# YuliangXiu/ICON

Measured on NVIDIA H100. Metric: M query-points/sec at 256^3 grid, higher is better.
Workload: dtype f32

## Files before the change

icon_b200/csrc/face_tree.cuh:

```cuda
#pragma once
#include <float.h>

#include "common.cuh"
#include "geom.cuh"

namespace icon {

__device__ __forceinline__ float box_dist2(V3 p, float4 lo, float4 hi) {
    const float dx = fmaxf(fmaxf(lo.x - p.x, p.x - hi.x), 0.f);
    const float dy = fmaxf(fmaxf(lo.y - p.y, p.y - hi.y), 0.f);
    const float dz = fmaxf(fmaxf(lo.z - p.z, p.z - hi.z), 0.f);
    return fmaf(dz, dz, fmaf(dy, dy, dx * dx));
}
__device__ __forceinline__ float box_far2(V3 p, float4 lo, float4 hi) {
    const float dx = fmaxf(fabsf(lo.x - p.x), fabsf(hi.x - p.x));
    const float dy = fmaxf(fabsf(lo.y - p.y), fabsf(hi.y - p.y));
    const float dz = fmaxf(fabsf(lo.z - p.z), fabsf(hi.z - p.z));
    return fmaf(dz, dz, fmaf(dy, dy, dx * dx));
}
__device__ __forceinline__ float warp_max(float v) {
    for (int o = 16; o; o >>= 1) v = fmaxf(v, __shfl_xor_sync(0xffffffffu, v, o));
    return v;
}
__device__ __forceinline__ float warp_min(float v) {
    for (int o = 16; o; o >>= 1) v = fminf(v, __shfl_xor_sync(0xffffffffu, v, o));
    return v;
}

static inline size_t tree_levels(FaceTree &t, int F) {
    t.F = F;
    int n = (F + 3) / 4, o = 0, l = 0;
    while (true) {
        t.lvl_cnt[l] = n; t.lvl_off[l] = o; o += n; ++l;
        if (n == 1) break;
        n = (n + 3) / 4;
    }
    t.nlevels = l;
    return (size_t)o;
}

__device__ __forceinline__ unsigned expand10(unsigned v) {
    v = (v * 0x00010001u) & 0xFF0000FFu;
    v = (v * 0x00000101u) & 0x0F00F00Fu;
    v = (v * 0x00000011u) & 0xC30C30C3u;
    v = (v * 0x00000005u) & 0x49249249u;
    return v;
}

__device__ __forceinline__ unsigned morton30(V3 p, V3 lo, float s) {
    auto qz = [s](float v, float l) { return (unsigned)fminf(fmaxf((v - l) * s, 0.f), 1023.f); };
    return (expand10(qz(p.x, lo.x)) << 2) | (expand10(qz(p.y, lo.y)) << 1) | expand10(qz(p.z, lo.z));
}

__device__ __forceinline__ V3 write_face_record(V3 a, V3 b, V3 c, float slack, float4 *__restrict__ tri,
                                                float4 *__restrict__ sph) {
    const V3 ab = sub3(b, a), ac = sub3(c, a);
    const V3 sc = mk3((a.x + b.x + c.x) / 3.f, (a.y + b.y + c.y) / 3.f, (a.z + b.z + c.z) / 3.f);
    const float ra = dot3(sub3(a, sc), sub3(a, sc)), rb = dot3(sub3(b, sc), sub3(b, sc)),
                rc = dot3(sub3(c, sc), sub3(c, sc));
    const float sr = sqrtf(fmaxf(ra, fmaxf(rb, rc))) * 1.0001f + slack;
    tri[0] = make_float4(a.x, a.y, a.z, ab.x);
    tri[1] = make_float4(ab.y, ab.z, ac.x, ac.y);
    tri[2] = make_float4(ac.z, 0.f, 0.f, 0.f);
    *sph = make_float4(sc.x, sc.y, sc.z, sr);
    return sc;
}

__device__ __forceinline__ void write_leaf_box(const FaceTree &t, int n) {
    float4 lo = make_float4(FLT_MAX, FLT_MAX, FLT_MAX, 0.f), hi = make_float4(-FLT_MAX, -FLT_MAX, -FLT_MAX, 0.f);
    for (int k = 4 * n; k < min(4 * n + 4, t.F); ++k) {
        const Tri tr = load_tri(t.tri_s + 3 * (size_t)k);
        const V3 vs[3] = {tr.a, mk3(tr.a.x + tr.ab.x, tr.a.y + tr.ab.y, tr.a.z + tr.ab.z),
                          mk3(tr.a.x + tr.ac.x, tr.a.y + tr.ac.y, tr.a.z + tr.ac.z)};
        for (int j = 0; j < 3; ++j) {
            lo.x = fminf(lo.x, vs[j].x); hi.x = fmaxf(hi.x, vs[j].x);
            lo.y = fminf(lo.y, vs[j].y); hi.y = fmaxf(hi.y, vs[j].y);
            lo.z = fminf(lo.z, vs[j].z); hi.z = fmaxf(hi.z, vs[j].z);
        }
    }
    t.nodes[2 * (size_t)n] = lo;
    t.nodes[2 * (size_t)n + 1] = hi;
}

__device__ __forceinline__ void write_parent_box(const FaceTree &t, int l, int n) {
    const float4 *child = t.nodes + 2 * (size_t)t.lvl_off[l - 1];
    float4 lo = make_float4(FLT_MAX, FLT_MAX, FLT_MAX, 0.f), hi = make_float4(-FLT_MAX, -FLT_MAX, -FLT_MAX, 0.f);
    for (int c = 4 * n; c < min(4 * n + 4, t.lvl_cnt[l - 1]); ++c) {
        const float4 a = child[2 * (size_t)c], b = child[2 * (size_t)c + 1];
        lo.x = fminf(lo.x, a.x); lo.y = fminf(lo.y, a.y); lo.z = fminf(lo.z, a.z);
        hi.x = fmaxf(hi.x, b.x); hi.y = fmaxf(hi.y, b.y); hi.z = fmaxf(hi.z, b.z);
    }
    t.nodes[2 * ((size_t)t.lvl_off[l] + n)] = lo;
    t.nodes[2 * ((size_t)t.lvl_off[l] + n) + 1] = hi;
}

struct ChunkSmem {
    float4 sph[32];
    float4 tri[32][3];
    int kk[32];
};
template <typename Id, int CAP>
struct WalkSmem : ChunkSmem {
    Id fr[2][CAP];
};

template <int PPW>
struct NearestFace {
    static constexpr int REP = 32 / PPW;
    const int lane;
    V3 p;
    float tol, tol_sup;
    float best = FLT_MAX;
    int bi = 0x7fffffff;
    float sb = 0.f, ub = 0.f;
    int staged = 0;

    __device__ __forceinline__ NearestFace(V3 p_, float tol_, float tol_sup_)
        : lane(threadIdx.x & 31), p(p_), tol(tol_), tol_sup(tol_sup_) {}

    __device__ __forceinline__ float sphere_bound(float d) const {
        const float b = d * rsqrtf(d) * 1.00001f + tol;
        return d > 0.f ? b : tol;
    }

    __device__ __forceinline__ void try_face(const float4 *rec, int f) {
        const Tri tr = load_tri(rec);
        const float d = tri_sqdist(p, tr.a, tr.ab, tr.ac);
        if (d < best || (d == best && f < bi)) { best = d; bi = f; }
    }

    __device__ __forceinline__ void descend(const FaceTree &t, V3 c) {
        int node = 0;
        for (int lvl = t.nlevels - 1; lvl > 0; --lvl) {
            const int ch = 4 * node + (lane & 3);
            float a = FLT_MAX;
            int ai = ch;
            if (ch < t.lvl_cnt[lvl - 1]) {
                const float4 *nb = t.nodes + 2 * ((size_t)t.lvl_off[lvl - 1] + ch);
                a = box_dist2(c, __ldg(nb), __ldg(nb + 1));
            }
            for (int o = 1; o <= 2; o <<= 1) {
                const float ob = __shfl_xor_sync(0xffffffffu, a, o);
                const int oi = __shfl_xor_sync(0xffffffffu, ai, o);
                if (ob < a || (ob == a && oi < ai)) { a = ob; ai = oi; }
            }
            node = __shfl_sync(0xffffffffu, ai, 0);
        }
        for (int k = 4 * node; k < min(4 * node + 4, t.F); ++k) try_face(t.tri_s + 3 * (size_t)k, __ldg(t.order + k));
    }

    __device__ __forceinline__ void start_scan(float ubw) {
        sb = sphere_bound(best);
        ub = ubw * 1.00001f + tol;
    }

    __device__ __forceinline__ void test(const FaceTree &t, int k, float4 s, const float4 *tr) {
        const float dx = p.x - s.x, dy = p.y - s.y, dz = p.z - s.z;
        const float dd = fmaf(dz, dz, fmaf(dy, dy, dx * dx));
        const float l = sb + s.w;
        if (dd > l * l) return;
        const float4 r0 = tr[0], r1 = tr[1], r2 = tr[2];
        const V3 ab = mk3(r0.w, r1.x, r1.y), ac = mk3(r1.z, r1.w, r2.x);
        const float S1 = fmaf(dz, ab.z, fmaf(dy, ab.y, dx * ab.x));
        const float T1 = fmaf(dz, ac.z, fmaf(dy, ac.y, dx * ac.x));
        const float M = fmaxf(fmaxf(-(S1 + T1), fmaf(2.f, S1, -T1)), fmaf(2.f, T1, -S1)) * (1.f / 3.f);
        const float g = dd - M - tol_sup;
        if (g > 0.f && g * g > best * dd * 1.0001f) return;
        const float d = tri_sqdist(p, mk3(r0.x, r0.y, r0.z), ab, ac);
        if (!(d <= best)) return;
        const int f = __ldg(t.order + k);
        if (d < best || f < bi) { best = d; bi = f; sb = sphere_bound(d); }
    }

    __device__ __forceinline__ void merge() {
#pragma unroll
        for (int o = PPW; o < 32; o <<= 1) {
            const float ob = __shfl_xor_sync(0xffffffffu, best, o);
            const int oi = __shfl_xor_sync(0xffffffffu, bi, o);
            if (ob < best || (ob == best && oi < bi)) { best = ob; bi = oi; }
        }
    }

    __device__ __forceinline__ void chunk(const FaceTree &t, ChunkSmem &S, int leaf, float4 wlo, float4 whi) {
        bool pass = false;
        int k = 0;
        float4 s = make_float4(0.f, 0.f, 0.f, 0.f);
        if (leaf >= 0) {
            k = 4 * leaf + (lane & 3);
            if (k < t.F) {
                s = __ldg(t.sph_s + k);
                const float l2 = ub + s.w;
                pass = box_dist2(mk3(s.x, s.y, s.z), wlo, whi) <= l2 * l2;
            }
        }
        const unsigned mask = __ballot_sync(0xffffffffu, pass);
        const int cnt = __popc(mask);
        staged += cnt;
        if (pass) {
            const int at = __popc(mask & ((1u << lane) - 1u));
            const float4 *tp = t.tri_s + 3 * (size_t)k;
            S.sph[at] = s;
            S.kk[at] = k;
            S.tri[at][0] = __ldg(tp); S.tri[at][1] = __ldg(tp + 1); S.tri[at][2] = __ldg(tp + 2);
        }
        __syncwarp();
        for (int j = lane / PPW; j < cnt; j += REP) test(t, S.kk[j], S.sph[j], &S.tri[j][0]);
        if (REP > 1) {
            merge();
            sb = sphere_bound(best);
        }
        ub = fminf(ub, warp_max(sb));
        __syncwarp();
    }

    template <typename Id>
    __device__ __forceinline__ void scan_leaves(const FaceTree &t, ChunkSmem &S, const Id *leaves, int n, float4 wlo,
                                                float4 whi) {
        for (int base = 0; base < n; base += 8) {
            const int slot = base + (lane >> 2);
            chunk(t, S, slot < n ? (int)leaves[slot] : -1, wlo, whi);
        }
    }

    __device__ __forceinline__ void scan_all(const FaceTree &t) {
        for (int k = lane / PPW; k < t.F; k += REP) test(t, k, __ldg(t.sph_s + k), t.tri_s + 3 * (size_t)k);
    }
};

template <typename Id, int CAP>
__device__ __forceinline__ bool tree_cull(const FaceTree &t, Id (&fr)[2][CAP], V3 c, float rw, float4 wlo, float4 whi,
                                          float tol, float &ubw, int &cur, int &n) {
    const int lane = threadIdx.x & 31;
    float ub2 = (ubw * 1.00001f + tol) * (ubw * 1.00001f + tol);
    cur = 0; n = 1;
    bool overflow = false;
    if (lane == 0) fr[0][0] = 0;
    __syncwarp();
    for (int lvl = t.nlevels - 1; lvl > 0 && !overflow; --lvl) {
        int nn = 0;
        float far2 = FLT_MAX;
        const int ccnt = t.lvl_cnt[lvl - 1];
        const float4 *nodes = t.nodes + 2 * (size_t)t.lvl_off[lvl - 1];
        for (int base = 0; base < n; base += 8) {
            const int slot = base + (lane >> 2);
            bool pass = false;
            int ch = 0;
            if (slot < n) {
                ch = 4 * (int)fr[cur][slot] + (lane & 3);
                if (ch < ccnt) {
                    const float4 lo = __ldg(nodes + 2 * (size_t)ch), hi = __ldg(nodes + 2 * (size_t)ch + 1);
                    const float gx = fmaxf(fmaxf(lo.x - whi.x, wlo.x - hi.x), 0.f);
                    const float gy = fmaxf(fmaxf(lo.y - whi.y, wlo.y - hi.y), 0.f);
                    const float gz = fmaxf(fmaxf(lo.z - whi.z, wlo.z - hi.z), 0.f);
                    pass = fmaf(gz, gz, fmaf(gy, gy, gx * gx)) <= ub2;
                    far2 = fminf(far2, box_far2(c, lo, hi));
                }
            }
            const unsigned mask = __ballot_sync(0xffffffffu, pass);
            const int at = nn + __popc(mask & ((1u << lane) - 1u));
            if (pass && at < CAP) fr[cur ^ 1][at] = (Id)ch;
            nn += __popc(mask);
        }
        overflow = nn > CAP;
        n = nn;
        cur ^= 1;
        const float l2 = sqrtf(warp_min(far2)) + rw;
        if (l2 < ubw) { ubw = l2; ub2 = (ubw * 1.00001f + tol) * (ubw * 1.00001f + tol); }
        __syncwarp();
    }
    return !overflow;
}

template <int PPW, typename Id, int CAP>
__device__ __forceinline__ int tree_nearest(const FaceTree &t, WalkSmem<Id, CAP> &S, NearestFace<PPW> &q, V3 c,
                                            float rw, float4 wlo, float4 whi) {
    q.descend(t, c);
    float ubw = warp_max(sqrtf(q.best));
    int cur, n;
    const bool ok = tree_cull(t, S.fr, c, rw, wlo, whi, q.tol, ubw, cur, n);
    q.start_scan(ubw);
    if (ok) q.scan_leaves(t, S, S.fr[cur], n, wlo, whi);
    else q.scan_all(t);
    q.merge();
    return n;
}

}
```

icon_b200/csrc/sdf.cu:

```cuda
#include <float.h>

#include <algorithm>
#include <mutex>
#include <type_traits>
#include <unordered_set>

#include "common.cuh"
#include "face_tree.cuh"
#include "geom.cuh"

namespace icon {

struct Calib {
    float r[9];
    float t[3];
};

__device__ __forceinline__ V3 load_point(const float *__restrict__ pts, int64_t sc, int64_t sn,
                                         int64_t i, const Calib &cb) {
    float px = pts[i * sn], py = pts[sc + i * sn], pz = pts[2 * sc + i * sn];
    V3 o;
    o.x = fmaf(cb.r[2], pz, fmaf(cb.r[1], py, cb.r[0] * px)) + cb.t[0];
    o.y = fmaf(cb.r[5], pz, fmaf(cb.r[4], py, cb.r[3] * px)) + cb.t[1];
    o.z = fmaf(cb.r[8], pz, fmaf(cb.r[7], py, cb.r[6] * px)) + cb.t[2];
    return o;
}

__device__ __forceinline__ void emit_record(V3 p, int bi, float best, int hits, const MeshView &m,
                                            float *__restrict__ rec, int32_t *__restrict__ face,
                                            int64_t idx) {
    Tri t = load_tri(m.tri + 3 * (size_t)bi);
    V3 n = cross3(t.ab, t.ac);
    float s = n.x * n.x + n.y * n.y + n.z * n.z;
    if (s == 0.f) s = 1e-6f;
    float inv = 1.0f / s;
    V3 w = sub3(p, t.a);
    V3 uw = cross3(t.ab, w), wv = cross3(w, t.ac);
    float b2 = (uw.x * n.x + uw.y * n.y + uw.z * n.z) * inv;
    float b1 = (wv.x * n.x + wv.y * n.y + wv.z * n.z) * inv;
    float b0 = 1.0f - b1 - b2;
    const float4 *at = m.attr + 6 * (size_t)bi;
    float4 a0 = __ldg(at), a1 = __ldg(at + 1), a2 = __ldg(at + 2), a3 = __ldg(at + 3),
           a4 = __ldg(at + 4), a5 = __ldg(at + 5);
    float nx = (a0.x * b0 + a0.w * b1 + a1.z * b2) * -1.f;
    float ny = (a0.y * b0 + a1.x * b1 + a1.w * b2) * 1.f;
    float nz = (a0.z * b0 + a1.y * b1 + a2.x * b2) * -1.f;
    float cx = a2.y * b0 + a3.x * b1 + a3.w * b2;
    float cy = a2.z * b0 + a3.y * b1 + a4.x * b2;
    float cz = a2.w * b0 + a3.z * b1 + a4.y * b2;
    float vv = a4.z * b0 + a4.w * b1 + a5.x * b2;
    float vis = vv >= 0.1f ? 1.f : 0.f;
    float dist = sqrtf(best) / sqrtf(3.0f);
    float sign = 2.0f * ((float)(hits & 1) - 0.5f);
    float sdf = dist * sign;
    float4 *r = (float4 *)(rec + 8 * idx);
    r[0] = make_float4(sdf, cx, cy, cz);
    r[1] = make_float4(nx, ny, nz, vis);
    if (face) face[idx] = bi;
}

constexpr int SW_T = 128;
constexpr int NBIN_AX = 128;
constexpr int NBIN = NBIN_AX * NBIN_AX * NBIN_AX;
__host__ __device__ constexpr int fr_cap(int ppw) { return ppw >= 16 ? 1024 : (ppw >= 4 ? 768 : 384); }

__device__ __forceinline__ unsigned spread7(unsigned v) {
    v = (v | (v << 16)) & 0x030000FFu;
    v = (v | (v << 8)) & 0x0300F00Fu;
    v = (v | (v << 4)) & 0x030C30C3u;
    v = (v | (v << 2)) & 0x09249249u;
    return v;
}

__device__ __forceinline__ int bin_of(V3 p) {
    const bool inside = p.x >= -1.f && p.x <= 1.f && p.y >= -1.f && p.y <= 1.f && p.z >= -1.f && p.z <= 1.f;
    if (!inside) return NBIN;
    const unsigned bx = min(NBIN_AX - 1, (int)((p.x + 1.f) * (NBIN_AX * 0.5f)));
    const unsigned by = min(NBIN_AX - 1, (int)((p.y + 1.f) * (NBIN_AX * 0.5f)));
    const unsigned bz = min(NBIN_AX - 1, (int)((p.z + 1.f) * (NBIN_AX * 0.5f)));
    return (int)(spread7(bx) | (spread7(by) << 1) | (spread7(bz) << 2));
}

__global__ void k_points_bin(const float *__restrict__ pts, int64_t sc, int64_t sn, int64_t N, Calib cb,
                             float4 *__restrict__ xyz4, int32_t *__restrict__ bid, int32_t *__restrict__ count) {
    const int64_t i = (int64_t)blockIdx.x * blockDim.x + threadIdx.x;
    const bool live = i < N;
    int b = -1;
    if (live) {
        const V3 p = load_point(pts, sc, sn, i, cb);
        const float in_cube = (p.x > -1.f && p.x < 1.f && p.y > -1.f && p.y < 1.f && p.z > -1.f && p.z < 1.f) ? 1.f : 0.f;
        xyz4[i] = make_float4(p.x, p.y, p.z, in_cube);
        b = bin_of(p);
        bid[i] = b;
    }
    const unsigned act = __ballot_sync(0xffffffffu, live);
    if (live) {
        const unsigned peers = __match_any_sync(act, b);
        if ((int)(threadIdx.x & 31) == __ffs(peers) - 1) atomicAdd(&count[b], __popc(peers));
    }
}

__global__ void k_points_scatter(const int32_t *__restrict__ bid, int64_t N, const int32_t *__restrict__ offset,
                                 int32_t *__restrict__ cursor, int32_t *__restrict__ perm) {
    const int64_t i = (int64_t)blockIdx.x * blockDim.x + threadIdx.x;
    const bool live = i < N;
    const int b = live ? bid[i] : -1;
    const unsigned act = __ballot_sync(0xffffffffu, live);
    if (live) {
        const unsigned peers = __match_any_sync(act, b);
        const int lane = threadIdx.x & 31, leader = __ffs(peers) - 1;
        int base = 0;
        if (lane == leader) base = atomicAdd(&cursor[b], __popc(peers));
        base = __shfl_sync(peers, base, leader);
        perm[offset[b] + base + __popc(peers & ((1u << lane) - 1u))] = (int32_t)i;
    }
}

#ifdef ICON_SDF_STATS
__device__ unsigned long long g_stats[8];
#define STAT(i, v) do { if (lane == 0) atomicAdd(&g_stats[i], (unsigned long long)(v)); } while (0)
#else
#define STAT(i, v) do { } while (0)
#endif

template <int PPW, bool BRICK>
using SdfSmem = typename std::conditional<BRICK, ChunkSmem, WalkSmem<unsigned short, fr_cap(PPW)>>::type;
template <int PPW, bool BRICK>
constexpr size_t sdf_smem_bytes() { return sizeof(SdfSmem<PPW, BRICK>) * (SW_T / 32); }

constexpr float BRICK_W = 2.0f / BRICK_AX;
constexpr float BRICK_HALF_DIAG = 0.0541266f;

__device__ __forceinline__ void brick_box(int b, float4 &lo, float4 &hi) {
    const int bx = b % BRICK_AX, by = (b / BRICK_AX) % BRICK_AX, bz = b / (BRICK_AX * BRICK_AX);
    lo = make_float4(-1.f + bx * BRICK_W, -1.f + by * BRICK_W, -1.f + bz * BRICK_W, 0.f);
    hi = make_float4(-1.f + (bx + 1) * BRICK_W, -1.f + (by + 1) * BRICK_W, -1.f + (bz + 1) * BRICK_W, 0.f);
}

__device__ __forceinline__ float leaf_key(const MeshView &m, int l, float4 lo, float4 hi) {
    const float4 a = __ldg(m.nodes + 2 * (size_t)l), z = __ldg(m.nodes + 2 * (size_t)l + 1);
    const float gx = fmaxf(fmaxf(a.x - hi.x, lo.x - z.x), 0.f);
    const float gy = fmaxf(fmaxf(a.y - hi.y, lo.y - z.y), 0.f);
    const float gz = fmaxf(fmaxf(a.z - hi.z, lo.z - z.z), 0.f);
    return fmaf(gz, gz, fmaf(gy, gy, gx * gx));
}

template <int PPW, bool BRICK>
__device__ __forceinline__ void sdf_warp(int64_t wid, SdfSmem<PPW, BRICK> &S, const float4 *__restrict__ xyz4,
                                         const int32_t *__restrict__ perm, int64_t N, const MeshView &m,
                                         float *__restrict__ rec, int32_t *__restrict__ face,
                                         int32_t *__restrict__ defer, int32_t *__restrict__ ndefer) {
    constexpr int REP = 32 / PPW;
    const int lane = threadIdx.x & 31;
    const int sub = lane % PPW, rep_id = lane / PPW;
    const int64_t pos0 = wid * PPW;
    const int64_t pos = pos0 + sub;
    if (pos0 >= N) return;
    const bool live = pos < N;
    const int64_t idx = perm[live ? pos : pos0];
    const float4 q = xyz4[idx];
    const V3 p = mk3(q.x, q.y, q.z);
    const V3 c = mk3(0.5f * (warp_min(p.x) + warp_max(p.x)), 0.5f * (warp_min(p.y) + warp_max(p.y)),
                     0.5f * (warp_min(p.z) + warp_max(p.z)));
    const float rw = warp_max(sqrtf(dot3(sub3(p, c), sub3(p, c)))) * 1.00001f + 1e-6f;
    const float4 wlo = make_float4(warp_min(p.x) - 1e-6f, warp_min(p.y) - 1e-6f, warp_min(p.z) - 1e-6f, 0.f);
    const float4 whi = make_float4(warp_max(p.x) + 1e-6f, warp_max(p.y) + 1e-6f, warp_max(p.z) + 1e-6f, 0.f);
    const MeshHeader h = *m.hdr;

    NearestFace<PPW> nf(p, 1e-6f, 1e-7f);
    if constexpr (BRICK) {
        bool ok = h.brick_built && !h.brick_overflow && c.x >= -1.f && c.x < 1.f && c.y >= -1.f && c.y < 1.f &&
                  c.z >= -1.f && c.z < 1.f;
        int b = 0;
        float4 blo, bhi;
        if (ok) {
            const int bx = min(BRICK_AX - 1, (int)((c.x + 1.f) * (BRICK_AX * 0.5f)));
            const int by = min(BRICK_AX - 1, (int)((c.y + 1.f) * (BRICK_AX * 0.5f)));
            const int bz = min(BRICK_AX - 1, (int)((c.z + 1.f) * (BRICK_AX * 0.5f)));
            b = (bz * BRICK_AX + by) * BRICK_AX + bx;
            brick_box(b, blo, bhi);
            ok = wlo.x >= blo.x && wlo.y >= blo.y && wlo.z >= blo.z && whi.x <= bhi.x && whi.y <= bhi.y && whi.z <= bhi.z;
        }
        if (!ok) {
            if (lane == 0) defer[atomicAdd(ndefer, 1)] = (int32_t)wid;
            return;
        }
        const int f = __ldg(m.bface + b);
        nf.try_face(m.tri + 3 * (size_t)f, f);
        nf.start_scan(fminf(warp_max(sqrtf(nf.best)), __ldg(m.bub + b)));
        STAT(0, 1);
        const int o1 = __ldg(m.boff + b + 1);
        for (int base = __ldg(m.boff + b); base < o1; base += 8) {
            const int slot = base + (lane >> 2);
            const int leaf = slot < o1 ? (int)__ldg(m.blist + slot) : -1;
            float key = 0.f;
            if (lane == 0) key = leaf_key(m, leaf, blo, bhi);
            if (__shfl_sync(0xffffffffu, key, 0) > nf.ub * nf.ub) break;
            STAT(2, min(8, o1 - base));
            nf.chunk(m, S, leaf, wlo, whi);
        }
        nf.merge();
    } else {
        const int n = tree_nearest(m, S, nf, c, rw, wlo, whi);
        STAT(0, 1); STAT(1, n > fr_cap(PPW) ? 1 : 0); STAT(2, n);
    }
    STAT(3, nf.staged);
    int hits = 0;
    if (!h.ray_overflow) {
        const float fy = (p.y - h.y0) * h.inv_cy, fz = (p.z - h.z0) * h.inv_cz;
        if (fy >= 0.f && fy < (float)RAY_GRID && fz >= 0.f && fz < (float)RAY_GRID) {
            const int cc = (int)fz * RAY_GRID + (int)fy;
            const int k0 = __ldg(m.roff + cc), k1 = __ldg(m.roff + cc + 1);
            for (int k = k0 + rep_id; k < k1; k += REP) {
                const int f = __ldg(m.rlist + k);
                if (__ldg(&m.rbox[2 * (size_t)f + 1].x) < p.x - 1e-3f) continue;
                const Tri tr = load_tri(m.tri + 3 * (size_t)f);
                hits += ray_hit_px(p, tr.a, tr.ab, tr.ac);
            }
        }
    } else {
        for (int f = rep_id; f < m.F; f += REP) {
            const Tri tr = load_tri(m.tri + 3 * (size_t)f);
            hits += ray_hit_px(p, tr.a, tr.ab, tr.ac);
        }
    }
    if (REP > 1) {
#pragma unroll
        for (int o = PPW; o < 32; o <<= 1) hits += __shfl_xor_sync(0xffffffffu, hits, o);
    }
    if (live && rep_id == 0) emit_record(p, nf.bi, nf.best, hits, m, rec, face, idx);
}

template <int PPW, bool BRICK>
__global__ void __launch_bounds__(SW_T) k_sdf_warp(const float4 *__restrict__ xyz4, const int32_t *__restrict__ perm,
                                                   int64_t N, MeshView m, float *__restrict__ rec,
                                                   int32_t *__restrict__ face, int32_t *__restrict__ defer,
                                                   int32_t *__restrict__ ndefer) {
    static_assert(!BRICK || PPW == 32, "brick lists serve dense lattices: 32 points per warp");
    extern __shared__ __align__(16) unsigned char smem_raw[];
    SdfSmem<PPW, BRICK> &S = reinterpret_cast<SdfSmem<PPW, BRICK> *>(smem_raw)[threadIdx.x >> 5];
    const bool listed = !BRICK && defer != nullptr;
    const int64_t nw = listed ? (int64_t)*ndefer : (N + PPW - 1) / PPW;
    for (int64_t i = (int64_t)blockIdx.x * (SW_T / 32) + (threadIdx.x >> 5); i < nw; i += (int64_t)gridDim.x * (SW_T / 32))
        sdf_warp<PPW, BRICK>(listed ? (int64_t)defer[i] : i, S, xyz4, perm, N, m, rec, face, defer, ndefer);
}

__global__ void k_brick_centres(MeshView m) {
    const int b = blockIdx.x * blockDim.x + threadIdx.x;
    if (b >= NBRICK) return;
    float4 lo, hi;
    brick_box(b, lo, hi);
    m.bxyz[b] = make_float4(0.5f * (lo.x + hi.x), 0.5f * (lo.y + hi.y), 0.5f * (lo.z + hi.z), 0.f);
    m.bperm[b] = b;
}

__global__ void __launch_bounds__(128) k_brick_count(MeshView m) {
    __shared__ int s_cnt;
    const int b = blockIdx.x;
    float4 lo, hi;
    brick_box(b, lo, hi);
    const float4 cc = m.bxyz[b];
    const Tri t = load_tri(m.tri + 3 * (size_t)m.bface[b]);
    const float d = tri_sqdist(mk3(cc.x, cc.y, cc.z), t.a, t.ab, t.ac);
    const float ub = (sqrtf(d) + BRICK_HALF_DIAG) * 1.00001f + 1e-6f, ub2 = ub * ub;
    if (threadIdx.x == 0) s_cnt = 0;
    __syncthreads();
    int cnt = 0;
    for (int l = threadIdx.x; l < m.lvl_cnt[0]; l += blockDim.x) cnt += leaf_key(m, l, lo, hi) <= ub2;
    for (int o = 16; o; o >>= 1) cnt += __shfl_xor_sync(0xffffffffu, cnt, o);
    if ((threadIdx.x & 31) == 0) atomicAdd(&s_cnt, cnt);
    __syncthreads();
    if (threadIdx.x == 0) {
        m.bub[b] = ub;
        m.boff[b] = s_cnt;
        if (s_cnt > BRICK_MAX_LEAVES) m.hdr->brick_overflow = 1;
        if (b == 0) m.boff[NBRICK] = 0;
    }
}

__global__ void __launch_bounds__(128) k_brick_fill(MeshView m, int64_t cap) {
    __shared__ float s_key[BRICK_MAX_LEAVES];
    __shared__ unsigned short s_leaf[BRICK_MAX_LEAVES];
    __shared__ int s_wcnt[4];
    if (m.hdr->brick_overflow || m.boff[NBRICK] > cap) return;
    const int b = blockIdx.x, o0 = m.boff[b], lane = threadIdx.x & 31, wib = threadIdx.x >> 5;
    float4 lo, hi;
    brick_box(b, lo, hi);
    const float ub = m.bub[b], ub2 = ub * ub;
    const int nleaf = m.lvl_cnt[0];
    int n = 0;
    for (int l0 = 0; l0 < nleaf; l0 += 128) {
        const int l = l0 + threadIdx.x;
        float key = 0.f;
        if (l < nleaf) key = leaf_key(m, l, lo, hi);
        const bool in = l < nleaf && key <= ub2;
        const unsigned bal = __ballot_sync(0xffffffffu, in);
        if (lane == 0) s_wcnt[wib] = __popc(bal);
        __syncthreads();
        int at = n + __popc(bal & ((1u << lane) - 1u));
        for (int w = 0; w < wib; ++w) at += s_wcnt[w];
        if (in) { s_key[at] = key; s_leaf[at] = (unsigned short)l; }
        n += s_wcnt[0] + s_wcnt[1] + s_wcnt[2] + s_wcnt[3];
        __syncthreads();
    }
    for (int i = threadIdx.x; i < n; i += blockDim.x) {
        const float k = s_key[i];
        int r = 0;
        for (int j = 0; j < n; ++j) {
            const float kj = s_key[j];
            r += kj < k || (kj == k && j < i);
        }
        m.blist[o0 + r] = s_leaf[i];
    }
}

__global__ void k_brick_done(MeshView m, int64_t cap) {
    if (m.boff[NBRICK] > cap) m.hdr->brick_overflow = 1;
    m.hdr->brick_built = 1;
}

__global__ void __launch_bounds__(256) k_sdf_brute(const float *__restrict__ pts, int64_t sc, int64_t sn,
                                                   int64_t N, Calib cb, MeshView m,
                                                   float *__restrict__ rec, int32_t *__restrict__ face) {
    __shared__ float4 tile[3 * 256];
    int64_t i = (int64_t)blockIdx.x * blockDim.x + threadIdx.x;
    bool live = i < N;
    V3 p = mk3(0.f, 0.f, 0.f);
    if (live) p = load_point(pts, sc, sn, i, cb);
    float best = FLT_MAX;
    int bi = 0, hits = 0;
    for (int f0 = 0; f0 < m.F; f0 += 256) {
        int nf = min(256, m.F - f0);
        __syncthreads();
        for (int k = threadIdx.x; k < 3 * nf; k += 256) tile[k] = m.tri[3 * (size_t)f0 + k];
        __syncthreads();
        if (live) {
            for (int k = 0; k < nf; ++k) {
                float4 r0 = tile[3 * k], r1 = tile[3 * k + 1], r2 = tile[3 * k + 2];
                V3 a = mk3(r0.x, r0.y, r0.z), ab = mk3(r0.w, r1.x, r1.y), ac = mk3(r1.z, r1.w, r2.x);
                float d = tri_sqdist(p, a, ab, ac);
                if (d < best) { best = d; bi = f0 + k; }
                hits += ray_hit_px(p, a, ab, ac);
            }
        }
    }
    if (live) emit_record(p, bi, best, hits, m, rec, face, i);
}

static int64_t g_sdf_ppw32_from = 6000000, g_sdf_ppw8_from = 300000;
static int g_sdf_ppw_force = 0;
static int g_sdf_bricks = 1;
static int64_t g_brick_max_entries = 0;

static std::mutex g_brick_mu;
static std::unordered_set<const void *> g_brick_ready;
static int64_t g_brick_builds = 0;

void bricks_forget(const MeshView &m) {
    std::lock_guard<std::mutex> lk(g_brick_mu);
    g_brick_ready.erase(m.hdr);
}

struct SdfWs {
    float4 *xyz4;
    int32_t *bid, *perm, *count, *offset;
    int32_t *defer, *ndefer;
    void *scan_ws;
};
static SdfWs carve_sdf(Carver &c, int64_t N) {
    SdfWs w;
    w.xyz4 = c.take<float4>((size_t)N);
    w.bid = c.take<int32_t>((size_t)N);
    w.perm = c.take<int32_t>((size_t)N);
    w.count = c.take<int32_t>(NBIN + 1);
    w.offset = c.take<int32_t>(NBIN + 1);
    w.defer = c.take<int32_t>((size_t)(N + 31) / 32);
    w.ndefer = c.take<int32_t>(1);
    w.scan_ws = c.take<char>(scan_ws_bytes(NBIN + 1));
    return w;
}

static int build_bricks(const MeshView &m, cudaStream_t stream) {
    const int64_t cap = g_brick_max_entries > 0 ? std::min(g_brick_max_entries, m.brick_cap) : m.brick_cap;
    k_brick_centres<<<NBRICK / 256, 256, 0, stream>>>(m);
    ICON_LAUNCHED();
    k_sdf_warp<1, false><<<NBRICK / (SW_T / 32), SW_T, sdf_smem_bytes<1, false>(), stream>>>(
        m.bxyz, m.bperm, NBRICK, m, m.brec, m.bface, nullptr, nullptr);
    ICON_LAUNCHED();
    k_brick_count<<<NBRICK, 128, 0, stream>>>(m);
    ICON_LAUNCHED();
    int rc = scan_exclusive_i32(m.boff, m.boff, NBRICK + 1, nullptr, m.scan_ws, stream);
    if (rc) return rc;
    k_brick_fill<<<NBRICK, 128, 0, stream>>>(m, cap);
    ICON_LAUNCHED();
    k_brick_done<<<1, 1, 0, stream>>>(m, cap);
    ICON_LAUNCHED();
    return ICON_OK;
}
size_t sdf_ws_bytes(int64_t N) {
    Carver c(nullptr);
    carve_sdf(c, N);
    return c.total();
}

Calib make_calib(const float *h) {
    Calib cb;
    for (int r = 0; r < 3; ++r) {
        for (int k = 0; k < 3; ++k) cb.r[3 * r + k] = h[4 * r + k];
        cb.t[r] = h[4 * r + 3];
    }
    return cb;
}

int run_sdf(const float *points, int64_t sc, int64_t sn, int64_t N, const float *h_calib,
            const MeshView &m, float *rec, int32_t *face, void *ws, float4 **xyz4_out,
            cudaStream_t stream) {
    Carver c(ws);
    SdfWs w = carve_sdf(c, N);
    Calib cb = make_calib(h_calib);
    profile_mark(0, stream);
    ICON_CUDA(cudaMemsetAsync(w.count, 0, sizeof(int32_t) * (NBIN + 1), stream));
    const unsigned nblk = (unsigned)((N + 255) / 256);
    k_points_bin<<<nblk, 256, 0, stream>>>(points, sc, sn, N, cb, w.xyz4, w.bid, w.count);
    ICON_LAUNCHED();
    int rc = scan_exclusive_i32(w.count, w.offset, NBIN + 1, nullptr, w.scan_ws, stream);
    if (rc) return rc;
    ICON_CUDA(cudaMemsetAsync(w.count, 0, sizeof(int32_t) * (NBIN + 1), stream));
    k_points_scatter<<<nblk, 256, 0, stream>>>(w.bid, N, w.offset, w.count, w.perm);
    ICON_LAUNCHED();
    static bool attr_set[ICON_MAX_DEVICES] = {};
    if (device_needs_setup(attr_set)) {
#define ICON_SDF_ATTR(P, B) ICON_CUDA(cudaFuncSetAttribute(k_sdf_warp<P, B>, cudaFuncAttributeMaxDynamicSharedMemorySize, \
                                                           (int)sdf_smem_bytes<P, B>()))
        ICON_SDF_ATTR(32, true); ICON_SDF_ATTR(32, false); ICON_SDF_ATTR(16, false); ICON_SDF_ATTR(8, false);
        ICON_SDF_ATTR(4, false); ICON_SDF_ATTR(2, false); ICON_SDF_ATTR(1, false);
#undef ICON_SDF_ATTR
    }
    profile_mark(1, stream);
    int ppw = N >= g_sdf_ppw32_from ? 32 : (N >= g_sdf_ppw8_from ? 8 : 1);
    if (g_sdf_ppw_force) ppw = g_sdf_ppw_force;
    const int wpb = SW_T / 32;
    const int64_t nwarps = (N + ppw - 1) / ppw;
    const unsigned nblk_w = (unsigned)((nwarps + wpb - 1) / wpb);
#define ICON_SDF_LAUNCH(P) k_sdf_warp<P, false><<<nblk_w, SW_T, sdf_smem_bytes<P, false>(), stream>>>( \
        w.xyz4, w.perm, N, m, rec, face, nullptr, nullptr)
    if (ppw == 32 && g_sdf_bricks) {
        bool build;
        {
            std::lock_guard<std::mutex> lk(g_brick_mu);
            build = g_brick_ready.insert(m.hdr).second;
        }
        if (build) {
            rc = build_bricks(m, stream);
            std::lock_guard<std::mutex> lk(g_brick_mu);
            if (rc) { g_brick_ready.erase(m.hdr); return rc; }
            ++g_brick_builds;
        }
        ICON_CUDA(cudaMemsetAsync(w.ndefer, 0, sizeof(int32_t), stream));
        k_sdf_warp<32, true><<<nblk_w, SW_T, sdf_smem_bytes<32, true>(), stream>>>(
            w.xyz4, w.perm, N, m, rec, face, w.defer, w.ndefer);
        ICON_LAUNCHED();
        const unsigned nblk_d = (unsigned)std::min<int64_t>(nblk_w, (int64_t)device_sm_count() * 16);
        k_sdf_warp<32, false><<<nblk_d, SW_T, sdf_smem_bytes<32, false>(), stream>>>(
            w.xyz4, w.perm, N, m, rec, face, w.defer, w.ndefer);
    } else {
        switch (ppw) {
            case 32: ICON_SDF_LAUNCH(32); break;
            case 16: ICON_SDF_LAUNCH(16); break;
            case 8: ICON_SDF_LAUNCH(8); break;
            case 4: ICON_SDF_LAUNCH(4); break;
            case 2: ICON_SDF_LAUNCH(2); break;
            default: ICON_SDF_LAUNCH(1); break;
        }
    }
#undef ICON_SDF_LAUNCH
    ICON_LAUNCHED();
    profile_mark(2, stream);
    if (xyz4_out) *xyz4_out = w.xyz4;
    return ICON_OK;
}

__global__ void k_points_only(const float *__restrict__ pts, int64_t sc, int64_t sn, int64_t N, Calib cb,
                              float4 *__restrict__ xyz4) {
    int64_t i = (int64_t)blockIdx.x * blockDim.x + threadIdx.x;
    if (i >= N) return;
    V3 p = load_point(pts, sc, sn, i, cb);
    float in_cube = (p.x > -1.f && p.x < 1.f && p.y > -1.f && p.y < 1.f && p.z > -1.f && p.z < 1.f) ? 1.f : 0.f;
    xyz4[i] = make_float4(p.x, p.y, p.z, in_cube);
}

int run_points_only(const float *points, int64_t sc, int64_t sn, int64_t N, const float *h_calib,
                    float4 *xyz4, cudaStream_t stream) {
    Calib cb = make_calib(h_calib);
    k_points_only<<<(unsigned)((N + 255) / 256), 256, 0, stream>>>(points, sc, sn, N, cb, xyz4);
    ICON_LAUNCHED();
    return ICON_OK;
}

}

using namespace icon;

#ifdef ICON_SDF_STATS
extern "C" int icon_debug_sdf_stats(unsigned long long *out, int reset) {
    cudaMemcpyFromSymbol(out, icon::g_stats, sizeof(unsigned long long) * 8);
    if (reset) { unsigned long long z[8] = {0}; cudaMemcpyToSymbol(icon::g_stats, z, sizeof(z)); }
    return 0;
}
#endif

extern "C" int icon_set_sdf_policy(int force_ppw, int64_t ppw8_from, int64_t ppw32_from) {
    ICON_CHECK_ARG(force_ppw >= 0 && force_ppw <= 32 && (force_ppw & (force_ppw - 1)) == 0, "icon_set_sdf_policy: ppw in {0,1,2,4,8,16,32}");
    icon::g_sdf_ppw_force = force_ppw;
    if (ppw8_from >= 0) icon::g_sdf_ppw8_from = ppw8_from;
    if (ppw32_from >= 0) icon::g_sdf_ppw32_from = ppw32_from;
    return ICON_OK;
}

extern "C" int icon_set_sdf_bricks(int enable, int64_t max_entries) {
    ICON_CHECK_ARG(enable == 0 || enable == 1, "icon_set_sdf_bricks: enable must be 0 or 1");
    icon::g_sdf_bricks = enable;
    icon::g_brick_max_entries = max_entries > 0 ? max_entries : 0;
    return ICON_OK;
}

extern "C" int icon_sdf_brick_info(const void *mesh_ws, int V, int F, int64_t *out) {
    ICON_CHECK_ARG(mesh_ws && out && V > 0 && F > 0, "icon_sdf_brick_info: bad argument");
    MeshView m = mesh_view(mesh_ws, V, F);
    MeshHeader h;
    int32_t total = 0;
    ICON_CUDA(cudaDeviceSynchronize());
    ICON_CUDA(cudaMemcpy(&h, m.hdr, sizeof(h), cudaMemcpyDeviceToHost));
    if (h.brick_built) ICON_CUDA(cudaMemcpy(&total, m.boff + NBRICK, sizeof(total), cudaMemcpyDeviceToHost));
    out[0] = h.brick_built;
    out[1] = h.brick_overflow;
    out[2] = total;
    out[3] = m.brick_cap;
    {
        std::lock_guard<std::mutex> lk(icon::g_brick_mu);
        out[4] = icon::g_brick_builds;
    }
    return ICON_OK;
}

extern "C" int icon_sdf_only(const float *points, int64_t stride_c, int64_t stride_n, int64_t N,
                             const float *h_calib, const void *mesh_ws, int V, int F, float *rec,
                             int32_t *face, void *ws, size_t ws_bytes, icon_stream_t stream_) {
    cudaStream_t stream = (cudaStream_t)stream_;
    ICON_CHECK_ARG(N >= 0 && N < (int64_t)INT32_MAX, "icon_sdf_only: N=%lld out of range", (long long)N);
    if (N == 0) return ICON_OK;
    ICON_CHECK_ARG(points && h_calib && mesh_ws && rec && ws, "icon_sdf_only: null pointer");
    if (ws_bytes < sdf_ws_bytes(N)) {
        set_error("icon_sdf_only: workspace %zu < %zu", ws_bytes, sdf_ws_bytes(N));
        return ICON_ENOSPC;
    }
    MeshView m = mesh_view(mesh_ws, V, F);
    return run_sdf(points, stride_c, stride_n, N, h_calib, m, rec, face, ws, nullptr, stream);
}

extern "C" int icon_sdf_bruteforce(const float *points, int64_t stride_c, int64_t stride_n, int64_t N,
                                   const float *h_calib, const void *mesh_ws, int V, int F, float *rec,
                                   int32_t *face, icon_stream_t stream_) {
    cudaStream_t stream = (cudaStream_t)stream_;
    if (N == 0) return ICON_OK;
    ICON_CHECK_ARG(points && h_calib && mesh_ws && rec, "icon_sdf_bruteforce: null pointer");
    MeshView m = mesh_view(mesh_ws, V, F);
    Calib cb = make_calib(h_calib);
    k_sdf_brute<<<(unsigned)((N + 255) / 256), 256, 0, stream>>>(points, stride_c, stride_n, N, cb, m, rec, face);
    ICON_LAUNCHED();
    return ICON_OK;
}
```

Before: 547.9.

## Add warp-wide linear-bound face culling for 32-point warps and raise min-blocks

For warps that hold 32 points, a per-warp linear model of each point's sphere bound is fitted over the brick (slope g and offset beta). Each candidate face is tested against it using a direction-projected triangle extent. Faces that are provably farther than every point's bound are dropped before staging, which cuts exact distance tests. This adds per-face sqrt/divide work and extra warp reductions per chunk. It also sets a minimum-blocks launch bound of 8 for PPW=32, which may cap registers and cause spills. Stats instrumentation is compiled only under a debug macro.

```diff
diff --git a/icon_b200/csrc/face_tree.cuh b/icon_b200/csrc/face_tree.cuh
--- a/icon_b200/csrc/face_tree.cuh
+++ b/icon_b200/csrc/face_tree.cuh
@@ -107,13 +107,24 @@
 template <int PPW>
 struct NearestFace {
     static constexpr int REP = 32 / PPW;
+    static constexpr bool CULL = PPW == 32;
     const int lane;
     V3 p;
     float tol, tol_sup;
     float best = FLT_MAX;
     int bi = 0x7fffffff;
     float sb = 0.f, ub = 0.f;
+    V3 g;
+    float beta = 0.f;
     int staged = 0;
+#ifdef ICON_SDF_STATS
+    int n_sph = 0, n_exact = 0, n_win = 0;
+    int n_dead = 0;
+    bool last_sph = false;
+#define NF_STAT(x) x
+#else
+#define NF_STAT(x)
+#endif
 
     __device__ __forceinline__ NearestFace(V3 p_, float tol_, float tol_sup_)
         : lane(threadIdx.x & 31), p(p_), tol(tol_), tol_sup(tol_sup_) {}
@@ -149,16 +160,36 @@
         for (int k = 4 * node; k < min(4 * node + 4, t.F); ++k) try_face(t.tri_s + 3 * (size_t)k, __ldg(t.order + k));
     }
 
-    __device__ __forceinline__ void start_scan(float ubw) {
+    __device__ __forceinline__ static float warp_sum(float v) {
+        for (int o = 16; o; o >>= 1) v += __shfl_xor_sync(0xffffffffu, v, o);
+        return v;
+    }
+    __device__ __forceinline__ V3 box_offset(float4 wlo, float4 whi) const {
+        return mk3(p.x - 0.5f * (wlo.x + whi.x), p.y - 0.5f * (wlo.y + whi.y), p.z - 0.5f * (wlo.z + whi.z));
+    }
+    __device__ __forceinline__ void update_beta(float4 wlo, float4 whi) {
+        beta = warp_max(fminf(sb, ub) - dot3(g, box_offset(wlo, whi)));
+    }
+
+    __device__ __forceinline__ void start_scan(float ubw, float4 wlo, float4 whi) {
         sb = sphere_bound(best);
         ub = ubw * 1.00001f + tol;
+        if (!CULL) return;
+        const V3 o = box_offset(wlo, whi);
+        const float sx = warp_sum(o.x * o.x), sy = warp_sum(o.y * o.y), sz = warp_sum(o.z * o.z);
+        const float bx = warp_sum(o.x * sb), by = warp_sum(o.y * sb), bz = warp_sum(o.z * sb);
+        auto slope = [](float num, float den) { return den > 0.f ? fminf(fmaxf(num / den, -1.f), 1.f) : 0.f; };
+        g = mk3(slope(bx, sx), slope(by, sy), slope(bz, sz));
+        update_beta(wlo, whi);
     }
 
     __device__ __forceinline__ void test(const FaceTree &t, int k, float4 s, const float4 *tr) {
         const float dx = p.x - s.x, dy = p.y - s.y, dz = p.z - s.z;
         const float dd = fmaf(dz, dz, fmaf(dy, dy, dx * dx));
         const float l = sb + s.w;
+        NF_STAT(last_sph = false);
         if (dd > l * l) return;
+        NF_STAT(++n_sph; last_sph = true);
         const float4 r0 = tr[0], r1 = tr[1], r2 = tr[2];
         const V3 ab = mk3(r0.w, r1.x, r1.y), ac = mk3(r1.z, r1.w, r2.x);
         const float S1 = fmaf(dz, ab.z, fmaf(dy, ab.y, dx * ab.x));
@@ -166,8 +197,10 @@
         const float M = fmaxf(fmaxf(-(S1 + T1), fmaf(2.f, S1, -T1)), fmaf(2.f, T1, -S1)) * (1.f / 3.f);
         const float g = dd - M - tol_sup;
         if (g > 0.f && g * g > best * dd * 1.0001f) return;
+        NF_STAT(++n_exact);
         const float d = tri_sqdist(p, mk3(r0.x, r0.y, r0.z), ab, ac);
         if (!(d <= best)) return;
+        NF_STAT(++n_win);
         const int f = __ldg(t.order + k);
         if (d < best || f < bi) { best = d; bi = f; sb = sphere_bound(d); }
     }
@@ -181,16 +214,35 @@
         }
     }
 
+    __device__ __forceinline__ bool beats(float4 s, float4 r0, float4 r1, float4 r2, float4 wlo, float4 whi) const {
+        const float vx = 0.5f * (wlo.x + whi.x) - s.x, vy = 0.5f * (wlo.y + whi.y) - s.y,
+                    vz = 0.5f * (wlo.z + whi.z) - s.z;
+        const float L = sqrtf(fmaf(vz, vz, fmaf(vy, vy, vx * vx)));
+        const float il = 1.f / L;
+        const float ex = vx * il, ey = vy * il, ez = vz * il;
+        const float S1 = fmaf(ez, r1.y, fmaf(ey, r1.x, ex * r0.w));
+        const float T1 = fmaf(ez, r2.x, fmaf(ey, r1.w, ex * r1.z));
+        const float he = fmaxf(fmaxf(-(S1 + T1), fmaf(2.f, S1, -T1)), fmaf(2.f, T1, -S1)) * (1.f / 3.f);
+        const float pr = fmaf(fabsf(ez - g.z), 0.5f * (whi.z - wlo.z),
+                              fmaf(fabsf(ey - g.y), 0.5f * (whi.y - wlo.y), fabsf(ex - g.x) * (0.5f * (whi.x - wlo.x))));
+        return L - he - pr - beta > tol + 1e-5f * (L + fabsf(he) + pr + fabsf(beta));
+    }
+
     __device__ __forceinline__ void chunk(const FaceTree &t, ChunkSmem &S, int leaf, float4 wlo, float4 whi) {
         bool pass = false;
         int k = 0;
-        float4 s = make_float4(0.f, 0.f, 0.f, 0.f);
+        float4 s = make_float4(0.f, 0.f, 0.f, 0.f), r0 = s, r1 = s, r2 = s;
         if (leaf >= 0) {
             k = 4 * leaf + (lane & 3);
             if (k < t.F) {
                 s = __ldg(t.sph_s + k);
                 const float l2 = ub + s.w;
                 pass = box_dist2(mk3(s.x, s.y, s.z), wlo, whi) <= l2 * l2;
+                if (CULL && pass) {
+                    const float4 *tp = t.tri_s + 3 * (size_t)k;
+                    r0 = __ldg(tp); r1 = __ldg(tp + 1); r2 = __ldg(tp + 2);
+                    pass = !beats(s, r0, r1, r2, wlo, whi);
+                }
             }
         }
         const unsigned mask = __ballot_sync(0xffffffffu, pass);
@@ -198,18 +250,25 @@
         staged += cnt;
         if (pass) {
             const int at = __popc(mask & ((1u << lane) - 1u));
-            const float4 *tp = t.tri_s + 3 * (size_t)k;
             S.sph[at] = s;
             S.kk[at] = k;
-            S.tri[at][0] = __ldg(tp); S.tri[at][1] = __ldg(tp + 1); S.tri[at][2] = __ldg(tp + 2);
+            if (!CULL) {
+                const float4 *tp = t.tri_s + 3 * (size_t)k;
+                r0 = __ldg(tp); r1 = __ldg(tp + 1); r2 = __ldg(tp + 2);
+            }
+            S.tri[at][0] = r0; S.tri[at][1] = r1; S.tri[at][2] = r2;
         }
         __syncwarp();
-        for (int j = lane / PPW; j < cnt; j += REP) test(t, S.kk[j], S.sph[j], &S.tri[j][0]);
+        for (int j = lane / PPW; j < cnt; j += REP) {
+            test(t, S.kk[j], S.sph[j], &S.tri[j][0]);
+            NF_STAT(if (REP == 1) n_dead += !__any_sync(0xffffffffu, last_sph));
+        }
         if (REP > 1) {
             merge();
             sb = sphere_bound(best);
         }
         ub = fminf(ub, warp_max(sb));
+        if (CULL) update_beta(wlo, whi);
         __syncwarp();
     }
 
@@ -278,7 +337,7 @@
     float ubw = warp_max(sqrtf(q.best));
     int cur, n;
     const bool ok = tree_cull(t, S.fr, c, rw, wlo, whi, q.tol, ubw, cur, n);
-    q.start_scan(ubw);
+    q.start_scan(ubw, wlo, whi);
     if (ok) q.scan_leaves(t, S, S.fr[cur], n, wlo, whi);
     else q.scan_all(t);
     q.merge();
diff --git a/icon_b200/csrc/sdf.cu b/icon_b200/csrc/sdf.cu
--- a/icon_b200/csrc/sdf.cu
+++ b/icon_b200/csrc/sdf.cu
@@ -118,9 +118,15 @@
 
 #ifdef ICON_SDF_STATS
 __device__ unsigned long long g_stats[8];
+__device__ unsigned *g_wstat;
+enum { WS_DEFER, WS_LEAVES, WS_STEPS, WS_STAGED, WS_SPH, WS_EXACT, WS_WIN, WS_RAY, WS_CYC_START, WS_CYC_C,
+       WS_CYC_RAY, WS_CYC_EMIT, WS_UB0, WS_UBEND, WS_LIST, WS_IDEAL_LEAVES, WS_IDEAL_FACES, WS_DEAD, WS_N = 20 };
 #define STAT(i, v) do { if (lane == 0) atomicAdd(&g_stats[i], (unsigned long long)(v)); } while (0)
+#define WSTAT(i, v) do { if (lane == 0 && g_wstat) g_wstat[(size_t)wid * WS_N + (i)] = (unsigned)(v); } while (0)
+#define WCLK(t) __syncwarp(); const long long t = clock64()
 #else
 #define STAT(i, v) do { } while (0)
+#define WSTAT(i, v) do { } while (0)
 #endif
 
 template <int PPW, bool BRICK>
@@ -168,6 +174,12 @@
     const MeshHeader h = *m.hdr;
 
     NearestFace<PPW> nf(p, 1e-6f, 1e-7f);
+#ifdef ICON_SDF_STATS
+    WCLK(t_start);
+    long long t_c = 0, t_ray = 0;
+    int st_leaves = 0, st_steps = 0, st_brick = -1;
+    float st_ub0 = 0.f;
+#endif
     if constexpr (BRICK) {
         bool ok = h.brick_built && !h.brick_overflow && c.x >= -1.f && c.x < 1.f && c.y >= -1.f && c.y < 1.f &&
                   c.z >= -1.f && c.z < 1.f;
@@ -183,12 +195,19 @@
         }
         if (!ok) {
             if (lane == 0) defer[atomicAdd(ndefer, 1)] = (int32_t)wid;
+            WSTAT(WS_DEFER, 1);
             return;
         }
         const int f = __ldg(m.bface + b);
         nf.try_face(m.tri + 3 * (size_t)f, f);
-        nf.start_scan(fminf(warp_max(sqrtf(nf.best)), __ldg(m.bub + b)));
+        nf.start_scan(fminf(warp_max(sqrtf(nf.best)), __ldg(m.bub + b)), wlo, whi);
         STAT(0, 1);
+#ifdef ICON_SDF_STATS
+        WCLK(t_c0);
+        t_c = t_c0;
+        st_brick = b;
+        st_ub0 = nf.ub;
+#endif
         const int o1 = __ldg(m.boff + b + 1);
         for (int base = __ldg(m.boff + b); base < o1; base += 8) {
             const int slot = base + (lane >> 2);
@@ -197,6 +216,10 @@
             if (lane == 0) key = leaf_key(m, leaf, blo, bhi);
             if (__shfl_sync(0xffffffffu, key, 0) > nf.ub * nf.ub) break;
             STAT(2, min(8, o1 - base));
+#ifdef ICON_SDF_STATS
+            st_leaves += min(8, o1 - base);
+            ++st_steps;
+#endif
             nf.chunk(m, S, leaf, wlo, whi);
         }
         nf.merge();
@@ -205,6 +228,10 @@
         STAT(0, 1); STAT(1, n > fr_cap(PPW) ? 1 : 0); STAT(2, n);
     }
     STAT(3, nf.staged);
+#ifdef ICON_SDF_STATS
+    WCLK(t_c1);
+    int st_ray = 0;
+#endif
     int hits = 0;
     if (!h.ray_overflow) {
         const float fy = (p.y - h.y0) * h.inv_cy, fz = (p.z - h.z0) * h.inv_cz;
@@ -216,6 +243,9 @@
                 if (__ldg(&m.rbox[2 * (size_t)f + 1].x) < p.x - 1e-3f) continue;
                 const Tri tr = load_tri(m.tri + 3 * (size_t)f);
                 hits += ray_hit_px(p, tr.a, tr.ab, tr.ac);
+#ifdef ICON_SDF_STATS
+                ++st_ray;
+#endif
             }
         }
     } else {
@@ -228,11 +258,58 @@
 #pragma unroll
         for (int o = PPW; o < 32; o <<= 1) hits += __shfl_xor_sync(0xffffffffu, hits, o);
     }
+#ifdef ICON_SDF_STATS
+    WCLK(t_ray0);
+    t_ray = t_ray0;
+#endif
     if (live && rep_id == 0) emit_record(p, nf.bi, nf.best, hits, m, rec, face, idx);
+#ifdef ICON_SDF_STATS
+    WCLK(t_end);
+    if (BRICK && st_brick >= 0) {
+        const float ube = nf.ub;
+        int il = 0, ifc = 0;
+        const int o0 = __ldg(m.boff + st_brick), o1 = __ldg(m.boff + st_brick + 1);
+        for (int s = o0 + lane; s < o1; s += 32) {
+            const int leaf = __ldg(m.blist + s);
+            const float4 a = __ldg(m.nodes + 2 * (size_t)leaf), z = __ldg(m.nodes + 2 * (size_t)leaf + 1);
+            const float gx = fmaxf(fmaxf(a.x - whi.x, wlo.x - z.x), 0.f);
+            const float gy = fmaxf(fmaxf(a.y - whi.y, wlo.y - z.y), 0.f);
+            const float gz = fmaxf(fmaxf(a.z - whi.z, wlo.z - z.z), 0.f);
+            if (fmaf(gz, gz, fmaf(gy, gy, gx * gx)) > ube * ube) continue;
+            ++il;
+            for (int k = 4 * leaf; k < min(4 * leaf + 4, m.F); ++k) {
+                const float4 s4 = __ldg(m.sph_s + k);
+                const float l2 = ube + s4.w;
+                ifc += box_dist2(mk3(s4.x, s4.y, s4.z), wlo, whi) <= l2 * l2;
+            }
+        }
+        const int s_sph = __reduce_add_sync(0xffffffffu, nf.n_sph), s_exact = __reduce_add_sync(0xffffffffu, nf.n_exact);
+        const int s_win = __reduce_add_sync(0xffffffffu, nf.n_win), s_ray = __reduce_add_sync(0xffffffffu, st_ray);
+        const int s_il = __reduce_add_sync(0xffffffffu, il), s_if = __reduce_add_sync(0xffffffffu, ifc);
+        WSTAT(WS_LEAVES, st_leaves);
+        WSTAT(WS_STEPS, st_steps);
+        WSTAT(WS_STAGED, nf.staged);
+        WSTAT(WS_SPH, s_sph);
+        WSTAT(WS_EXACT, s_exact);
+        WSTAT(WS_WIN, s_win);
+        WSTAT(WS_RAY, s_ray);
+        WSTAT(WS_CYC_START, t_c - t_start);
+        WSTAT(WS_CYC_C, t_c1 - t_c);
+        WSTAT(WS_CYC_RAY, t_ray - t_c1);
+        WSTAT(WS_CYC_EMIT, t_end - t_ray);
+        WSTAT(WS_UB0, __float_as_uint(st_ub0));
+        WSTAT(WS_UBEND, __float_as_uint(ube));
+        WSTAT(WS_LIST, o1 - o0);
+        WSTAT(WS_IDEAL_LEAVES, s_il);
+        WSTAT(WS_IDEAL_FACES, s_if);
+        WSTAT(WS_DEAD, nf.n_dead);
+    }
+    if (!BRICK && defer != nullptr) { STAT(4, 1); STAT(5, t_end - t_start); }
+#endif
 }
 
 template <int PPW, bool BRICK>
-__global__ void __launch_bounds__(SW_T) k_sdf_warp(const float4 *__restrict__ xyz4, const int32_t *__restrict__ perm,
+__global__ void __launch_bounds__(SW_T, PPW == 32 ? 8 : 0) k_sdf_warp(const float4 *__restrict__ xyz4, const int32_t *__restrict__ perm,
                                                    int64_t N, MeshView m, float *__restrict__ rec,
                                                    int32_t *__restrict__ face, int32_t *__restrict__ defer,
                                                    int32_t *__restrict__ ndefer) {
@@ -507,6 +584,11 @@
     if (reset) { unsigned long long z[8] = {0}; cudaMemcpyToSymbol(icon::g_stats, z, sizeof(z)); }
     return 0;
 }
+
+extern "C" int icon_debug_sdf_warp_stats(unsigned *dev_buf) {
+    cudaMemcpyToSymbol(icon::g_wstat, &dev_buf, sizeof(dev_buf));
+    return 0;
+}
 #endif
 
 extern "C" int icon_set_sdf_policy(int force_ppw, int64_t ppw8_from, int64_t ppw32_from) {
```

After: 589.5 (median of 6 runs). 7.6% higher.
